# Lumina-Group/libzkp

Hardware: AMD Instinct MI355X
Metric: proofs/sec (whole node) + ms/proof p50, 4096-proof mixed batch (range / equality / membership / improvement) per MI355X (higher is better)
Workload: dtype u32/u64 integer limbs (10x25.5-bit GF(2^255-19), BN254 Fq on 9x29-bit limbs in the MSM loops and 10x26-bit elsewhere, 8x32-bit Fr and scalars mod l, 2x64-bit f128)

## Files before the change

libzkp_amd/csrc/edg.h:

```cpp
#pragma once
#include "bp_steps.h"

namespace zkp {

constexpr uint32_t EDG_WBITS = 16, EDG_NWIN = 16, EDG_NENT = 1u << 15, EDG_DIGW = 8, EDG_NWIN_U64 = 5;
constexpr uint32_t EDG_SLOT_W = 32, EDG_ENTRY_W = 24;
constexpr uint32_t EDG_SEG = 64, EDG_NSEG = EDG_NENT / EDG_SEG, EDG_INV = 8;

struct EdgGeom { uint32_t wbits, nwin, nwin_u64, nent, nseg; };
constexpr uint32_t EDG_WBITS_MIN = 10, EDG_WBITS_MAX = 16;
ZKP_HD constexpr EdgGeom edg_geom(uint32_t wbits) {
    return EdgGeom{wbits, sc_signed_ndigits(wbits, 254), sc_signed_ndigits(wbits, 65), 1u << (wbits - 1), (1u << (wbits - 1)) / EDG_SEG};
}
static_assert(edg_geom(EDG_WBITS).nwin == EDG_NWIN && edg_geom(EDG_WBITS).nwin_u64 == EDG_NWIN_U64 && edg_geom(EDG_WBITS).nent == EDG_NENT &&
              edg_geom(EDG_WBITS).nseg == EDG_NSEG, "the EDG_* constants are the radix-2^16 geometry");
static_assert(edg_geom(EDG_WBITS_MIN).nwin <= 2 * DIGW, "digit rows hold 2 * DIGW digits");
ZKP_HD constexpr size_t edg_table_words(const EdgGeom& g) { return (size_t)NBASE * g.nwin * g.nent * EDG_SLOT_W; }
ZKP_HD constexpr size_t edg_slot(const EdgGeom& g, uint32_t b, uint32_t w, uint32_t e) { return (((size_t)b * g.nwin + w) * g.nent + e) * EDG_SLOT_W; }
ZKP_HD constexpr size_t edg_table_words() { return edg_table_words(edg_geom(EDG_WBITS)); }
ZKP_HD constexpr size_t edg_slot(uint32_t b, uint32_t w, uint32_t e) { return edg_slot(edg_geom(EDG_WBITS), b, w, e); }

ZKP_HD inline ge_niels edg_unpack(const uint32_t e[EDG_ENTRY_W]) {
    ge_niels n; n.ypx = fe_fromwords(e); n.ymx = fe_fromwords(e + 8); n.xy2d = fe_fromwords(e + 16);
    return n;
// ... 36 lines not shown
ZKP_HD inline void edg_step_bases(const uint32_t* gens, uint32_t* bases, uint32_t b) { edg_step_bases(edg_geom(EDG_WBITS), gens, bases, b); }
ZKP_HD inline void edg_step_starts(const uint32_t* bases, uint32_t* starts, uint32_t bw) { edg_step_starts(edg_geom(EDG_WBITS), bases, starts, bw); }
ZKP_HD inline void edg_step_fill(const uint32_t* bases, const uint32_t* starts, uint32_t* table, uint32_t bw, uint32_t s) { edg_step_fill(edg_geom(EDG_WBITS), bases, starts, table, bw, s); }
ZKP_HD inline fe edg_fe_invert(const fe& z) {
    fe t = fe_pow22523(z);
    t = fe_sq(fe_sq(fe_sq(t)));
    return fe_mul(t, fe_mul(fe_sq(z), z));
}
ZKP_HD inline void edg_step_affine(uint32_t* table, size_t group) {
    uint32_t* q0 = table + group * EDG_INV * EDG_SLOT_W;
    fe pre[EDG_INV];
    fe run = fe_one();
    for (uint32_t i = 0; i < EDG_INV; i++) {
        fe z; ZKP_UNROLL for (int k = 0; k < 10; k++) z.v[k] = q0[(size_t)i * EDG_SLOT_W + 20 + k];
        pre[i] = run; run = fe_mul(run, z);
    }
    fe inv = edg_fe_invert(run);
    const fe d2 = fe_const_d2();
    for (uint32_t i = EDG_INV; i-- > 0;) {
        uint32_t* q = q0 + (size_t)i * EDG_SLOT_W;
        fe X, Y, Z; ZKP_UNROLL for (int k = 0; k < 10; k++) { X.v[k] = q[k]; Y.v[k] = q[10 + k]; Z.v[k] = q[20 + k]; }
        const fe zi = fe_mul(inv, pre[i]);
        inv = fe_mul(inv, Z);
        const fe x = fe_mul(X, zi), y = fe_mul(Y, zi);
        fe_towords(q, fe_add(y, x));
        fe_towords(q + 8, fe_sub(y, x));
        fe_towords(q + 16, fe_mul(fe_mul(x, y), d2));
        ZKP_UNROLL for (int k = EDG_ENTRY_W; k < (int)EDG_SLOT_W; k++) q[k] = 0;
    }
}
ZKP_HD inline bool edg_niels_equals(const ge& p, const uint32_t e[EDG_ENTRY_W]) {
    const ge_niels n = edg_unpack(e);
    return fe_eq(fe_add(p.Y, p.X), fe_mul(n.ypx, p.Z)) && fe_eq(fe_sub(p.Y, p.X), fe_mul(n.ymx, p.Z));
}
ZKP_HD inline ge edg_point_of(const uint32_t e[EDG_ENTRY_W]) {
    const ge_niels n = edg_unpack(e);
    ge p; p.X = fe_carry(fe_sub(n.ypx, n.ymx)); p.Y = fe_carry(fe_add(n.ypx, n.ymx)); p.Z = fe_zero(); p.Z.v[0] = 2;
    p.T = fe_mul(p.X, p.Y); p.X = fe_carry(fe_add(p.X, p.X)); p.Y = fe_carry(fe_add(p.Y, p.Y)); p.Z.v[0] = 4;
    return p;
}
ZKP_HD inline bool edg_step_check(const EdgGeom& g, const uint32_t* table, const uint32_t* gens, uint32_t b, uint32_t w, uint32_t e) {
    const uint32_t* cur = table + edg_slot(g, b, w, e);
    if (e + 1 < g.nent) {
        const ge sum = ge_madd(edg_point_of(cur), edg_unpack(table + edg_slot(g, b, w, 0)));
        if (!edg_niels_equals(sum, cur + EDG_SLOT_W)) return false;
    } else if (w + 1 < g.nwin) {
        if (!edg_niels_equals(ge_dbl(edg_point_of(cur)), table + edg_slot(g, b, w + 1, 0))) return false;
    }
    if (w == 0 && e == 0 && !edg_niels_equals(ld_ge(gens, b, 0, 1), cur)) return false;
    return true;
}
ZKP_HD inline bool edg_step_check(const uint32_t* table, const uint32_t* gens, uint32_t b, uint32_t w, uint32_t e) { return edg_step_check(edg_geom(EDG_WBITS), table, gens, b, w, e); }

}
```

libzkp_amd/csrc/edg_kernels.hip:

```cpp
#include "edg_launch.h"
#include "msm_kernel.h"

struct EdGather {
    static constexpr uint32_t ACC_W = GE_W, DIG_PER_WORD = 2;
    static __device__ __forceinline__ int32_t digit(uint32_t word, uint32_t w) { return (int32_t)(int16_t)(word >> (16 * (w & 1u))); }
    using Acc = ge;
    static __device__ __forceinline__ Acc identity() { return ge_identity(); }
    static constexpr uint32_t GATHER_WAVES = 3; static constexpr int GATHER_PREFETCH = 2;
    static constexpr uint32_t GATHER_W = EDG_ENTRY_W, GATHER_STRIDE = EDG_SLOT_W, GATHER_PRIO = 0;
    using GAcc = ge;
    static __device__ __forceinline__ GAcc to_gather(const ge& a) { return a; }
    static __device__ __forceinline__ ge from_gather(const GAcc& a) { return a; }
    static __device__ __forceinline__ GAcc accumulate_entry(const GAcc& acc, int32_t d, const uint32_t* e) { return edg_accumulate(acc, d, e); }
    static __device__ __forceinline__ void store(uint32_t* p, uint32_t idx, uint32_t row, uint32_t rows, const Acc& a) { st_ge(p, idx, row, rows, a); }
    static __device__ __forceinline__ Acc load(const uint32_t* p, uint32_t idx, uint32_t row, uint32_t rows) { return ld_ge(p, idx, row, rows); }
    static __device__ __forceinline__ Acc add(const Acc& a, const Acc& b) { return ge_add(a, b); }
};
template __global__ void k_msm_gather<EdGather>(MsmView, uint32_t, uint32_t);
struct EdGatherPrio : EdGather { static constexpr uint32_t GATHER_PRIO = 1; };
template __global__ void k_msm_gather<EdGatherPrio>(MsmView, uint32_t, uint32_t);

uint32_t edg_msm_rows_per_block() { return 256; }
uint32_t edg_msm_blocks_per_cu() {
    int occ = 0;
    if (hipOccupancyMaxActiveBlocksPerMultiprocessor(&occ, k_msm_gather<EdGather>, 256, gather_lds_bytes<EdGather>()) != hipSuccess) { (void)hipGetLastError(); return 0; }
    return occ > 0 ? (uint32_t)occ : 0;
}
void edg_launch_msm(const MsmView& m, uint32_t ngroups, uint32_t nblocks, hipStream_t st, bool raised) {
    const uint32_t grid = ((nblocks + 7) / 8) * 8;
    if (raised) k_msm_gather<EdGatherPrio><<<grid, 256, gather_lds_bytes<EdGather>(), st>>>(m, ngroups, nblocks);
    else k_msm_gather<EdGather><<<grid, 256, gather_lds_bytes<EdGather>(), st>>>(m, ngroups, nblocks);
}

template <uint32_t WB> __global__ void __launch_bounds__(64) k_edg_bases(const uint32_t* gens, uint32_t* bases) {
    const uint32_t b = blockIdx.x * 64 + threadIdx.x;
    if (b < NBASE) edg_step_bases(edg_geom(WB), gens, bases, b);
}
template <uint32_t WB> __global__ void __launch_bounds__(64) k_edg_starts(const uint32_t* bases, uint32_t* starts) {
    constexpr EdgGeom g = edg_geom(WB);
    const uint32_t bw = blockIdx.x * 64 + threadIdx.x;
    if (bw < NBASE * g.nwin) edg_step_starts(g, bases, starts, bw);
}
template <uint32_t WB> __global__ void __launch_bounds__(256) k_edg_fill(const uint32_t* bases, const uint32_t* starts, uint32_t* table) {
    constexpr EdgGeom g = edg_geom(WB);
    const uint32_t t = blockIdx.x * 256 + threadIdx.x;
    if (t < NBASE * g.nwin * g.nseg) edg_step_fill(g, bases, starts, table, t / g.nseg, t % g.nseg);
}
template <uint32_t WB> __global__ void __launch_bounds__(256) k_edg_affine(uint32_t* table) {
    constexpr EdgGeom g = edg_geom(WB);
    const size_t grp = (size_t)blockIdx.x * 256 + threadIdx.x;
    if (grp < (size_t)NBASE * g.nwin * g.nent / EDG_INV) edg_step_affine(table, grp);
}
template <uint32_t WB> __global__ void __launch_bounds__(256) k_edg_check(const uint32_t* table, const uint32_t* gens, int* bad) {
    constexpr EdgGeom g = edg_geom(WB);
    const size_t t = (size_t)blockIdx.x * 256 + threadIdx.x;
    if (t >= (size_t)NBASE * g.nwin * g.nent) return;
    const uint32_t e = (uint32_t)(t % g.nent), bw = (uint32_t)(t / g.nent);
    if (!edg_step_check(g, table, gens, bw / g.nwin, bw % g.nwin, e)) atomicAdd(bad, 1);
}
template <uint32_t WB> void edg_launch_build_at(const uint32_t* d_gens, uint32_t* d_table, uint32_t* d_scratch, int* d_bad, hipStream_t st) {
    constexpr EdgGeom g = edg_geom(WB);
    uint32_t* bases = d_scratch;
    uint32_t* starts = d_scratch + (size_t)NBASE * g.nwin * GE_W;
    k_edg_bases<WB><<<(NBASE + 63) / 64, 64, 0, st>>>(d_gens, bases);
    k_edg_starts<WB><<<(NBASE * g.nwin + 63) / 64, 64, 0, st>>>(bases, starts);
    k_edg_fill<WB><<<(NBASE * g.nwin * g.nseg + 255) / 256, 256, 0, st>>>(bases, starts, d_table);
    const size_t groups = (size_t)NBASE * g.nwin * g.nent / EDG_INV, slots = (size_t)NBASE * g.nwin * g.nent;
    k_edg_affine<WB><<<(uint32_t)((groups + 255) / 256), 256, 0, st>>>(d_table);
    k_edg_check<WB><<<(uint32_t)((slots + 255) / 256), 256, 0, st>>>(d_table, d_gens, d_bad);
}
size_t edg_build_scratch_words(const EdgGeom& g) { return (size_t)NBASE * g.nwin * (g.nseg + 1) * GE_W; }
void edg_launch_build(const EdgGeom& g, const uint32_t* d_gens, uint32_t* d_table, uint32_t* d_scratch, int* d_bad, hipStream_t st) {
    switch (g.wbits) {
        case 10: edg_launch_build_at<10>(d_gens, d_table, d_scratch, d_bad, st); break;
        case 11: edg_launch_build_at<11>(d_gens, d_table, d_scratch, d_bad, st); break;
        case 12: edg_launch_build_at<12>(d_gens, d_table, d_scratch, d_bad, st); break;
        case 13: edg_launch_build_at<13>(d_gens, d_table, d_scratch, d_bad, st); break;
        case 14: edg_launch_build_at<14>(d_gens, d_table, d_scratch, d_bad, st); break;
        case 15: edg_launch_build_at<15>(d_gens, d_table, d_scratch, d_bad, st); break;
        default: edg_launch_build_at<16>(d_gens, d_table, d_scratch, d_bad, st); break;
    }
}
```

libzkp_amd/csrc/edg_launch.h:

```cpp
#pragma once
#include <hip/hip_runtime.h>
#include "edg.h"

uint32_t edg_msm_rows_per_block();
uint32_t edg_msm_blocks_per_cu();
void edg_launch_msm(const zkp::MsmView& m, uint32_t ngroups, uint32_t nblocks, hipStream_t st, bool raised = false);
void edg_launch_build(const zkp::EdgGeom& g, const uint32_t* d_gens, uint32_t* d_table, uint32_t* d_scratch, int* d_bad, hipStream_t st);
size_t edg_build_scratch_words(const zkp::EdgGeom& g);
void edg_launch_sum(const zkp::ReduceView& R, uint32_t* sums, hipStream_t st);
```

libzkp_amd/csrc/zkp_hip.hip:

```cpp
#include <hip/hip_runtime.h>
#include <mutex>
#include <memory>
#include <algorithm>
#include <map>
#include <array>
#include <type_traits>
#include <atomic>
#include <thread>
#include <condition_variable>
#include <functional>
#include <deque>
#include <new>
#include <exception>
#include <cstring>
#include <string>
#include <vector>
#include <cstdio>
#include <cstdlib>
#include <cmath>
#include <chrono>
#include <sys/random.h>
#include "bp_layout.h"
#include "g16_steps.h"
#include "sha256_host.h"
// ... 201 lines not shown
    std::vector<void*> owned;
    DevScope() = default;
    DevScope(const DevScope&) = delete;
    DevScope& operator=(const DevScope&) = delete;
    ~DevScope() { release(); }
    void release() { if (!owned.empty()) dev_scope_quiesce(); for (void* q : owned) dev_pool().give(q); owned.clear(); }
    template <class T> hipError_t alloc(T** out, size_t bytes) {
        void* q = nullptr;
        const hipError_t e = dev_pool().take(&q, bytes ? bytes : 1);
        if (e == hipSuccess) owned.push_back(q);
        *out = static_cast<T*>(q);
        return e;
    }
};
struct Quiesce { bool armed = true; ~Quiesce() { if (armed) (void)hipDeviceSynchronize(); } };

struct DevLayout {
    uint16_t *slot_base = nullptr, *chunk_begin = nullptr, *chunk_win0 = nullptr, *chunk_nwin = nullptr, *target_chunk_begin = nullptr;
    uint8_t* slot_nwin = nullptr;
    uint32_t nslots = 0, nchunks = 0, ntargets = 0, max_chunk_windows = 0, max_target_chunks = 0;
    uint64_t adds_per_row = 0;
    uint32_t *steps = nullptr, *chunk_step0 = nullptr;
};
constexpr int MAXT = 8;
struct LayoutSet { std::vector<DevLayout> cand; uint32_t max_chunks = 0; };

struct SubBatch {
    hipStream_t stream = nullptr;
    hipEvent_t start = nullptr, done = nullptr;
    hipStream_t side = nullptr;
    hipEvent_t side_go = nullptr, side_done = nullptr;
    bool used = false;
    bool borrowed = false;
    void* ws = nullptr;
    uint32_t capM = 0, capC = 0, cap_chunks = 0;
};
constexpr uint32_t NSLOTS = 2;

struct G16State; struct StarkState; struct VfyState; struct BatchState;
struct Device {
    int index = 0, hip_dev = 0;
    std::mutex mu;
    bool ready = false;
    uint64_t generation = 0;
    int num_cu = 256;
    int msm_prio_now = 0;
    hipStream_t stream = nullptr;
    uint32_t* d_edg_table = nullptr;
    EdgGeom edg = {0, 0, 0, 0, 0};
    bool bp_ready = false;
    int edg_blocks_per_cu = 3;
    struct Family { LayoutSet p1, rd[6]; bool ready = false; };
    Family fam[4];
    LayoutSet p2, ct;
    uint32_t max_chunks = 0;
    SubBatch sub[NSLOTS];
    uint32_t next_slot = 0;
    DevPool pool;
    G16State* g16 = nullptr; StarkState* stark = nullptr; VfyState* vfy = nullptr; BatchState* batch = nullptr;
    bool profiling = false;
    struct KProf {
        std::vector<std::pair<hipEvent_t, hipEvent_t>> ev_pool; size_t ev_used = 0;
        double ms = 0; uint64_t launches = 0, adds = 0;
    };
    KProf prof[3];
    struct HostCounter { double ms = 0; uint64_t a = 0, b = 0; };
    HostCounter host[ZKP_HIP_COUNTER_VERIFY_MIXED - ZKP_HIP_COUNTER_G16_VERIFY + 1];
    HostCounter& counter(int which) { return host[which - ZKP_HIP_COUNTER_G16_VERIFY]; }
    struct BpLocaliseCounter { double ms = 0; uint64_t failed_checks = 0, segment_checks = 0, jobs_again = 0; } bp_localise;
    struct CompositesCounter { double ms = 0; uint64_t composites = 0, malformed = 0, envelopes = 0; } composites;
    uint64_t stark_verify_resident = 0;
    struct Trace* trace = nullptr;
    struct ShardWorker* worker = nullptr;
};
struct ShardWorker {
    struct Job { std::function<void()> fn; bool done = false; };
    using Ticket = std::shared_ptr<Job>;
    std::mutex mu; std::condition_variable cv;
    std::deque<Ticket> queue;
    std::thread th;
    ShardWorker() : th([this]() { run(); }) { th.detach(); }
    void run() {
        for (;;) {
            Ticket t;
            { std::unique_lock<std::mutex> lk(mu); cv.wait(lk, [this]() { return !queue.empty(); }); t = queue.front(); queue.pop_front(); }
            t->fn();
            { std::lock_guard<std::mutex> lk(mu); t->done = true; }
            cv.notify_all();
        }
    }
    Ticket post(std::function<void()> f) {
        Ticket t = std::make_shared<Job>(); t->fn = std::move(f);
        { std::lock_guard<std::mutex> lk(mu); queue.push_back(t); }
        cv.notify_all();
        return t;
    }
    void wait(const Ticket& t) { std::unique_lock<std::mutex> lk(mu); cv.wait(lk, [&]() { return t->done; }); }
};
std::mutex g_worker_create_mu;
int prof_begin(Device::KProf& K, hipStream_t st, hipEvent_t* e1);
void prof_end(Device::KProf& K, hipStream_t st, hipEvent_t e1, uint64_t adds);
struct Registry {
    std::mutex mu;
    std::vector<Device*> shards;
    bool hooked = false;
};
Registry& registry() { static Registry* r = new Registry(); return *r; }
thread_local Device* t_dev = nullptr;
thread_local int t_sel = 0;
thread_local bool t_sel_chosen = false;
Device& dev() { return *t_dev; }
DevPool& dev_pool() { return dev().pool; }
void dev_scope_quiesce() { if (dev().stream) (void)hipStreamSynchronize(dev().stream); }
uint32_t g_budget_request = 0;
int env_int(const char* name, int dflt) { const char* v = getenv(name); return v && *v ? atoi(v) : dflt; }
int stream_priority(int level) {
    int least = 0, greatest = 0; (void)hipDeviceGetStreamPriorityRange(&least, &greatest);
    return level == 0 ? greatest : level == 2 ? least : (least + greatest) / 2;
}
int bp_priority_level() { static const int v = env_int("ZKP_HIP_BP_PRIORITY", 1); return v; }
int stark_priority_level() { static const int v = env_int("ZKP_HIP_STARK_PRIORITY", 1); return v; }
int g16_priority_level() { static const int v = env_int("ZKP_HIP_G16_PRIORITY", 2); return v; }

int prof_begin(Device::KProf& K, hipStream_t st, hipEvent_t* e1) {
    *e1 = nullptr;
    if (!dev().profiling) return 0;
    if (K.ev_used == K.ev_pool.size()) { hipEvent_t a, b; HIP_TRY(hipEventCreate(&a)); HIP_TRY(hipEventCreate(&b)); K.ev_pool.push_back({a, b}); }
    HIP_TRY(hipEventRecord(K.ev_pool[K.ev_used].first, st));
    *e1 = K.ev_pool[K.ev_used].second; K.ev_used++;
    return 0;
}
void prof_end(Device::KProf& K, hipStream_t st, hipEvent_t e1, uint64_t adds) {
    if (!e1) return;
    (void)hipEventRecord(e1, st); K.launches++; K.adds += adds;
}

struct Trace {
    struct Rec { const char* name; hipStream_t st; hipEvent_t a, b; };
    std::vector<Rec> recs;
    std::vector<hipEvent_t> pool; size_t used = 0;
    hipEvent_t origin = nullptr; bool have_origin = false;
    std::string path;
    hipEvent_t take() { if (used == pool.size()) { hipEvent_t e = nullptr; (void)hipEventCreate(&e); pool.push_back(e); } return pool[used++]; }
};
Trace* trace_state() {
    Device& D = dev();
    if (D.trace) return D.trace->path.empty() ? nullptr : D.trace;
    D.trace = new Trace();
    const char* v = getenv("ZKP_HIP_TRACE");
    if (v && *v) D.trace->path = v;
    return D.trace->path.empty() ? nullptr : D.trace;
}
void trace_origin(hipStream_t st) {
    Trace* T = trace_state(); if (!T) return;
    if (!T->origin) (void)hipEventCreate(&T->origin);
    (void)hipEventRecord(T->origin, st); T->have_origin = true;
}
struct TraceMark {
    Trace* T; Trace::Rec r;
    TraceMark(const char* name, hipStream_t st) : T(trace_state()) { if (T) { r = {name, st, T->take(), T->take()}; (void)hipEventRecord(r.a, st); } }
    ~TraceMark() { if (T) { (void)hipEventRecord(r.b, r.st); T->recs.push_back(r); } }
};
#define ZKP_TRACED(name, st, ...) do { TraceMark tm_(name, st); __VA_ARGS__; } while (0)
void trace_dump() {
    Trace* T = trace_state(); if (!T || T->recs.empty()) return;
    (void)hipDeviceSynchronize();
    FILE* f = fopen(T->path.c_str(), "a");
    if (f) {
        std::map<hipStream_t, int> ids;
        fputs("[", f);
        bool first = true;
        for (auto& r : T->recs) {
            float ta = 0, tb = 0;
            if (!T->have_origin || hipEventElapsedTime(&ta, T->origin, r.a) != hipSuccess || hipEventElapsedTime(&tb, T->origin, r.b) != hipSuccess) continue;
            const int id = ids.emplace(r.st, (int)ids.size()).first->second;
// ... 144 lines not shown
    if (!strcmp(v, "lazy")) { *lazy = true; return 0; }
    return fail(ZKP_HIP_E_ARGUMENT, "ZKP_HIP_ED_TABLES must be eager or lazy");
}
int build_edg_table() {
    Device& D = dev();
    if (D.d_edg_table) return 0;
    EdgTables& R = edg_tables();
    std::lock_guard<std::mutex> registry_lock(R.mu);
    {
        const uint32_t occ = edg_msm_blocks_per_cu();
        D.edg_blocks_per_cu = occ ? (int)occ : 3;
    }
    for (auto& e : R.v) if (e.hip_dev == D.hip_dev && e.refs > 0) { e.refs++; D.d_edg_table = e.table; D.edg = e.geom; return 0; }
    uint32_t wbits = 0;
    int rc = choose_ed_radix(&wbits);
    if (rc) return rc;
    const EdgGeom g = edg_geom(wbits);
    ge gens[NBASE]; host_generators(gens);
    std::vector<uint32_t> gw((size_t)NBASE * GE_W);
    for (uint32_t b = 0; b < NBASE; b++) st_ge(gw.data(), b, 0, 1, gens[b]);
    uint32_t *d_gens = nullptr, *d_scratch = nullptr; int* d_bad = nullptr;
    const size_t table_bytes = edg_table_words(g) * 4, scratch_bytes = edg_build_scratch_words(g) * 4;
    if (hipMalloc(&D.d_edg_table, table_bytes) != hipSuccess) {
        (void)hipGetLastError(); D.d_edg_table = nullptr;
        char msg[200]; snprintf(msg, sizeof msg, "out of device memory allocating the %llu MB of generator window tables (radix 2^%u)", (unsigned long long)(table_bytes >> 20), wbits);
        return fail(ZKP_HIP_E_RUNTIME, msg);
    }
    auto drop = [&]() { (void)hipFree(d_gens); (void)hipFree(d_scratch); (void)hipFree(d_bad); };
    auto give_up = [&](int code, const std::string& m) { drop(); (void)hipFree(D.d_edg_table); D.d_edg_table = nullptr; return fail(code, m); };
    hipError_t e = hipMalloc(&d_gens, gw.size() * 4);
    if (e == hipSuccess) e = hipMalloc(&d_scratch, scratch_bytes);
    if (e == hipSuccess) e = hipMalloc(&d_bad, sizeof(int));
    if (e == hipSuccess) e = hipMemcpyAsync(d_gens, gw.data(), gw.size() * 4, hipMemcpyHostToDevice, D.stream);
    if (e == hipSuccess) e = hipMemsetAsync(d_bad, 0, sizeof(int), D.stream);
    if (e != hipSuccess) return give_up(ZKP_HIP_E_RUNTIME, std::string("generator tables: ") + hipGetErrorString(e));
    edg_launch_build(g, d_gens, D.d_edg_table, d_scratch, d_bad, D.stream);
    int bad = -1;
    e = hipGetLastError();
    if (e == hipSuccess) e = hipMemcpyAsync(&bad, d_bad, sizeof(int), hipMemcpyDeviceToHost, D.stream);
    if (e == hipSuccess) e = hipStreamSynchronize(D.stream);
    if (e != hipSuccess) return give_up(ZKP_HIP_E_RUNTIME, std::string("generator tables: ") + hipGetErrorString(e));
    if (bad != 0) { char msg[160]; snprintf(msg, sizeof msg, "generator window tables failed their self-check (%d inconsistent slots)", bad); return give_up(ZKP_HIP_E_RUNTIME, msg); }
    drop();
    D.edg = g;
    R.v.push_back({D.hip_dev, D.d_edg_table, 1, g});
    return 0;
}
int ensure_bp() {
    Device& D = dev();
    if (D.bp_ready) return 0;
    int rc;
    if ((rc = build_edg_table())) return rc;
    D.max_chunks = 0;
    if ((rc = upload_set(D.p2, targets_phase2((uint8_t)D.edg.nwin)))) return rc;
    if ((rc = upload_set(D.ct, targets_ctask((uint8_t)D.edg.nwin, (uint8_t)D.edg.nwin_u64)))) return rc;
    D.max_chunks = D.p2.max_chunks;
    if ((rc = ensure_family(6))) return rc;
    D.bp_ready = true;
    return 0;
}

int init_device() {
    Device& D = dev();
    if (D.ready) return 0;
    bool lazy = false;
    int rc = ed_tables_lazy(&lazy);
    if (rc) return rc;
    hipDeviceProp_t prop; HIP_TRY(hipGetDeviceProperties(&prop, D.hip_dev));
    D.num_cu = prop.multiProcessorCount > 0 ? prop.multiProcessorCount : 256;
    if (!D.stream) HIP_TRY(hipStreamCreateWithFlags(&D.stream, hipStreamNonBlocking));
    if (!lazy && (rc = ensure_bp())) return rc;
    D.ready = true;
    return 0;
}
void release_sub(SubBatch& sb) {
    if (sb.ws) (void)hipFree(sb.ws);
    for (hipEvent_t e : {sb.start, sb.done, sb.side_go, sb.side_done}) if (e) (void)hipEventDestroy(e);
    if (!sb.borrowed) { if (sb.stream) (void)hipStreamDestroy(sb.stream); if (sb.side) (void)hipStreamDestroy(sb.side); }
    sb = SubBatch();
}
int ensure_sub(SubBatch& sb, SubBatch* share = nullptr) {
    if (sb.stream) return 0;
    SubBatch t;
    int rc = 0;
    if (share && share != &sb) {
        if ((rc = ensure_sub(*share))) return rc;
        t.stream = share->stream; t.side = share->side; t.borrowed = true;
    } else {
        hipError_t e = hipStreamCreateWithPriority(&t.stream, hipStreamNonBlocking, stream_priority(bp_priority_level()));
        if (e == hipSuccess) e = hipStreamCreateWithPriority(&t.side, hipStreamNonBlocking, stream_priority(bp_priority_level()));
        if (e != hipSuccess) { release_sub(t); return fail(ZKP_HIP_E_RUNTIME, std::string("hipStreamCreateWithPriority: ") + hipGetErrorString(e)); }
    }
    for (hipEvent_t* e : {&t.start, &t.done, &t.side_go, &t.side_done}) {
        const hipError_t err = hipEventCreateWithFlags(e, hipEventDisableTiming);
        if (err != hipSuccess) { *e = nullptr; release_sub(t); return fail(ZKP_HIP_E_RUNTIME, std::string("hipEventCreateWithFlags: ") + hipGetErrorString(err)); }
    }
    sb.start = t.start; sb.done = t.done; sb.side_go = t.side_go; sb.side_done = t.side_done;
    sb.side = t.side; sb.borrowed = t.borrowed; sb.stream = t.stream;
    return 0;
}

extern "C" void zkp_hip_shutdown(void);
void batch_release_all();
void stark_release_all();
int register_shards_locked(Registry& R, const int* devices, uint32_t count, bool add, const char* bad_index) {
    int ndev = 0;
    if (hipGetDeviceCount(&ndev) != hipSuccess || ndev == 0)
        return fail(ZKP_HIP_E_RUNTIME, "zkp_hip_init: no HIP device available (this library has no CPU fallback)");
    for (uint32_t k = 0; k < count; k++) if (devices[k] < 0 || devices[k] >= ndev) return fail(ZKP_HIP_E_ARGUMENT, bad_index);
// ... 100 lines not shown
        rc = verify_fan_out(shards, F.holds.empty() ? nullptr : F.holds.data(), n, F.prefix.empty() ? nullptr : F.prefix.data(), F.unit, F.min_jobs, slice, &fanned);
        if (rc || fanned) return rc;
    }
    Bind bind;
    if ((rc = bind.open())) return rc;
    return slice(0, n);
}
struct EnvelopeUpload {
    DevScope mem;
    uint8_t *d_in = nullptr, *d_ok = nullptr; uint32_t* d_len = nullptr; uint64_t *d_p0 = nullptr, *d_p1 = nullptr;
    int open(uint64_t n, const uint8_t* proofs, uint64_t stride, const uint32_t* lens, const uint64_t* p0 = nullptr, const uint64_t* p1 = nullptr) {
        hipStream_t st = dev().stream;
        HIP_TRY(mem.alloc(&d_in, stride * n)); HIP_TRY(mem.alloc(&d_len, 4 * n)); HIP_TRY(mem.alloc(&d_ok, n));
        if (p0) HIP_TRY(mem.alloc(&d_p0, 8 * n));
        if (p1) HIP_TRY(mem.alloc(&d_p1, 8 * n));
        HIP_TRY(hipMemcpyAsync(d_in, proofs, stride * n, hipMemcpyHostToDevice, st));
        HIP_TRY(hipMemcpyAsync(d_len, lens, 4 * n, hipMemcpyHostToDevice, st));
        if (p0) HIP_TRY(hipMemcpyAsync(d_p0, p0, 8 * n, hipMemcpyHostToDevice, st));
        if (p1) HIP_TRY(hipMemcpyAsync(d_p1, p1, 8 * n, hipMemcpyHostToDevice, st));
        return 0;
    }
};

struct Ws {
    JobBuf J; BpView V; CtView T;
    uint32_t *partial, *ct_partial, *ct_enc, *sums, *ct_sums;
    uint64_t* ct_off;
    int* flag;
};
size_t align_up(size_t x) { return (x + 255) & ~(size_t)255; }

size_t carve(uint8_t* base, uint32_t M, uint32_t C, uint32_t max_chunks, Ws* w) {
    size_t off = 0;
    auto take = [&](size_t bytes) { uint8_t* p = base ? base + off : nullptr; off += align_up(bytes); return p; };
    const size_t W = (size_t)8 * 4 * M;
    const size_t WD = (size_t)DIGW * 4 * M;
    Ws t{};
    t.J.v = (uint64_t*)take(8ull * M); t.J.seed_ix = (uint32_t*)take(4ull * M); t.J.proof_ix = (uint32_t*)take(4ull * M);
    t.J.bl_plus = (int32_t*)take(4ull * M); t.J.bl_minus = (int32_t*)take(4ull * M); t.J.kind = (uint8_t*)take(M);
    t.J.proof_off = (uint64_t*)take(8ull * M); t.J.commit_off = (uint64_t*)take(8ull * M);
    t.J.ct_v = (uint64_t*)take(8ull * C); t.J.ct_seed_ix = (uint32_t*)take(4ull * C); t.J.ct_bl_ix = (uint32_t*)take(4ull * C); t.J.ct_off = (uint64_t*)take(8ull * C);
    t.V.wbits = dev().edg.wbits; t.T.wbits = dev().edg.wbits;
    t.V.M = M; t.V.v = t.J.v; t.V.seed_ix = t.J.seed_ix; t.V.proof_ix = t.J.proof_ix; t.V.bl_plus = t.J.bl_plus; t.V.bl_minus = t.J.bl_minus;
    t.V.kind = t.J.kind; t.V.proof_off = t.J.proof_off; t.V.commit_off = t.J.commit_off;
    t.V.tape = (uint32_t*)take(W * TAPE_SLOTS); t.V.gamma = (uint32_t*)take(W);
    t.V.d1 = (uint32_t*)take(WD * P1_NSLOTS); t.V.d2 = (uint32_t*)take(WD * P2_NSLOTS); t.V.dr = (uint32_t*)take(WD * PR_NSLOTS);
    t.V.yinvpow = (uint32_t*)take(W * 64); t.V.ypq = (uint32_t*)take(W * 32); t.V.r0 = (uint32_t*)take(W * 64); t.V.r1 = (uint32_t*)take(W * 64);
    t.V.pp = (uint32_t*)take(W * 192); t.V.ab = (uint32_t*)take(W * 256); t.V.gh = (uint32_t*)take(W * 128);
    t.V.scal = (uint32_t*)take(W * SC_NUM); t.V.tstate = (uint32_t*)take(4ull * 52 * M); t.V.enc = (uint32_t*)take(W * 3);
    t.partial = (uint32_t*)take((size_t)max_chunks * GE_W * 4 * M);
    t.sums = (uint32_t*)take((size_t)3 * GE_W * 4 * M);
    t.T.C = C; t.T.v = t.J.ct_v; t.T.seed_ix = t.J.ct_seed_ix; t.T.bl_ix = t.J.ct_bl_ix;
    t.T.digits = (uint32_t*)take((size_t)2 * DIGW * 4 * C);
    t.ct_partial = (uint32_t*)take((size_t)(dev().ct.max_chunks ? dev().ct.max_chunks : 2) * GE_W * 4 * C);
    t.ct_enc = (uint32_t*)take((size_t)8 * 4 * C);
    t.ct_sums = (uint32_t*)take((size_t)GE_W * 4 * C);
    t.ct_off = t.J.ct_off;
    t.flag = (int*)take(256);
    if (w) *w = t;
    return off;
}

int ensure_workspace(SubBatch& sb, uint32_t M, uint32_t C) {
    if (M <= sb.capM && C <= sb.capC && dev().max_chunks <= sb.cap_chunks && sb.ws) return 0;
    if (sb.ws) { HIP_TRY(hipDeviceSynchronize()); HIP_TRY(hipFree(sb.ws)); sb.ws = nullptr; }
    const uint32_t nm = M > sb.capM ? M : sb.capM, nc = C > sb.capC ? C : sb.capC;
    const size_t bytes = carve(nullptr, nm, nc, dev().max_chunks, nullptr);
    HIP_TRY(hipMalloc(&sb.ws, bytes));
    sb.capM = nm; sb.capC = nc; sb.cap_chunks = dev().max_chunks;
    return 0;
}

int launch_msm(const DevLayout& D, uint32_t rows, const uint32_t* digits, uint32_t* partial, hipStream_t st) {
    MsmView m; m.rows = rows; m.nslots = D.nslots; m.nchunks = D.nchunks; m.table = dev().d_edg_table; m.digits = digits;
    m.slot_base = D.slot_base; m.slot_scalar = nullptr; m.slot_nwin = D.slot_nwin; m.chunk_begin = D.chunk_begin; m.chunk_win0 = D.chunk_win0; m.chunk_nwin = D.chunk_nwin; m.partial = partial; m.acc_init = nullptr;
    hipEvent_t e1 = nullptr;
    int rc = prof_begin(dev().prof[0], st, &e1);
    if (rc) return rc;
    {
        const EdgGeom& g = dev().edg;
        m.nwin = g.nwin; m.nent = g.nent; m.digw = DIGW; m.slot_ent = g.nwin * g.nent; m.uneven = 0;
        m.steps = D.steps; m.chunk_step0 = D.chunk_step0;
        const uint32_t tb = edg_msm_rows_per_block(), ngroups = (rows + tb - 1) / tb, nblocks = D.nchunks * ngroups;
        ZKP_TRACED("k_msm_gather<EdGather>", st, edg_launch_msm(m, ngroups, nblocks, st, dev().msm_prio_now != 0));
    }
    prof_end(dev().prof[0], st, e1, D.adds_per_row * rows);
    return 0;
}
void launch_sum_ed(const ReduceView& R, uint32_t* sums, hipStream_t st) {
    k_sum_t<EdMsm, ED_SUM_ROWS, ED_SUM_TB><<<dim3((R.rows + ED_SUM_ROWS - 1) / ED_SUM_ROWS, R.ntargets), ED_SUM_TB, 0, st>>>(R, sums);
}
int launch_reduce(const DevLayout& D, uint32_t rows, const uint32_t* partial, uint32_t* sums, uint32_t* enc, const uint64_t* out_off, uint8_t* out, hipStream_t st) {
    ReduceView R; R.rows = rows; R.ntargets = D.ntargets; R.partial = partial; R.target_chunk_begin = D.target_chunk_begin;
    R.enc = enc; R.out_off = out_off; R.out = out; R.corr = nullptr;
    ZKP_TRACED("k_sum_t<EdMsm>", st, launch_sum_ed(R, sums, st));
    ZKP_TRACED("k_encode", st, k_encode<<<dim3((rows + TW - 1) / TW, D.ntargets), TW, 0, st>>>(R, sums));
    return 0;
}
int msm_and_encode(const LayoutSet& S, uint32_t rows, const uint32_t* digits, uint32_t* partial, uint32_t* sums, uint32_t* enc, const uint64_t* out_off, uint8_t* out, hipStream_t st) {
    const DevLayout& D = pick_layout(S, rows);
    int rc = launch_msm(D, rows, digits, partial, st);
    if (rc) return rc;
    return launch_reduce(D, rows, partial, sums, enc, out_off, out, st);
}

int run_pipeline(const Ws& w, uint32_t M, uint32_t C, hipStream_t st, SubBatch& lane) {
    int rc;
    const dim3 gj((M + TB - 1) / TB), gw((M + TW - 1) / TW);
    const uint32_t n = w.V.n, lg = w.V.lg;
    const Device::Family& F = dev().fam[lg - 3];
    const bool forked = C != 0 && M != 0;
    if (C) {
        hipStream_t cs = forked ? lane.side : st;
        if (forked) { HIP_TRY(hipEventRecord(lane.side_go, st)); HIP_TRY(hipStreamWaitEvent(cs, lane.side_go, 0)); }
        ZKP_TRACED("k_ctask", cs, k_ctask<<<(C + TB - 1) / TB, TB, 0, cs>>>(w.T));
        if ((rc = msm_and_encode(dev().ct, C, w.T.digits, w.ct_partial, w.ct_sums, w.ct_enc, w.ct_off, w.V.out, cs))) return rc;
        if (forked) HIP_TRY(hipEventRecord(lane.side_done, cs));
    }
    if (M == 0) { HIP_TRY(hipGetLastError()); return 0; }
    ZKP_TRACED("k_tape", st, k_tape<<<dim3(gj.x, tape_slots(n) + 1), TB, 0, st>>>(w.V));
    if ((rc = msm_and_encode(F.p1, M, w.V.d1, w.partial, w.sums, w.V.enc, nullptr, nullptr, st))) return rc;
    ZKP_TRACED("k_transcript1", st, k_transcript1<<<gw, TW, 0, st>>>(w.V));
    ZKP_TRACED("k_poly", st, k_poly<<<dim3(gj.x, n), TB, 0, st>>>(w.V));
    ZKP_TRACED("k_poly_sum", st, k_poly_sum<<<(M + 7) / 8, TW, 0, st>>>(w.V));
    if ((rc = msm_and_encode(dev().p2, M, w.V.d2, w.partial, w.sums, w.V.enc, nullptr, nullptr, st))) return rc;
    ZKP_TRACED("k_transcript2", st, k_transcript2<<<gw, TW, 0, st>>>(w.V));
    ZKP_TRACED("k_lr_init", st, k_lr_init<<<dim3(gj.x, n), TB, 0, st>>>(w.V));
    for (uint32_t r = 0; r < lg; r++) {
        ZKP_TRACED("k_round_prep", st, k_round_prep<<<dim3(gj.x, n), TB, 0, st>>>(w.V, r));
        ZKP_TRACED("k_round_sum", st, k_round_sum<<<gw, TW, 0, st>>>(w.V, r));
        if ((rc = msm_and_encode(F.rd[r], M, w.V.dr, w.partial, w.sums, w.V.enc, nullptr, nullptr, st))) return rc;
        ZKP_TRACED("k_transcript_round", st, k_transcript_round<<<gw, TW, 0, st>>>(w.V, r));
    }
    if (forked) HIP_TRY(hipStreamWaitEvent(st, lane.side_done, 0));
    HIP_TRY(hipGetLastError());
    return 0;
}

__global__ void k_any_failed(const int32_t* status, uint32_t n, int* flag) {
    const uint32_t i = blockIdx.x * blockDim.x + threadIdx.x;
    if (i < n && status[i] != 0) atomicOr(flag, 1);
}

int prove_range_device_locked(uint64_t n, const uint64_t* d_value, const uint64_t* d_min, const uint64_t* d_max, uint32_t lg,
                              const uint8_t* d_seeds, uint8_t* d_out, uint64_t stride, uint32_t* d_out_len, int32_t* d_status,
                              hipStream_t st, int* any_failed, int slot_hint = -1) {
    if (n == 0) { if (any_failed) *any_failed = 0; return 0; }
    { int rcn = check_batch_size(n); if (rcn) return rcn; }
    if (stride < range_envelope_bytes(lg)) return fail(ZKP_HIP_E_ARGUMENT, "stride is smaller than the proof (1478 bytes for n_bits = 64)");
    int rc;
    if ((rc = ensure_family(lg))) return rc;
    uint32_t slot = 0;
    if (slot_hint >= 0) slot = (uint32_t)slot_hint % NSLOTS;
    else {
        SubBatch& s0 = dev().sub[0];
        if (s0.used && hipEventQuery(s0.done) == hipErrorNotReady) { slot = 1 + dev().next_slot % (NSLOTS - 1); dev().next_slot++; }
        (void)hipGetLastError();
    }
    SubBatch& sb = dev().sub[slot];
    if ((rc = ensure_sub(sb, &dev().sub[0]))) return rc;
    HIP_TRY(hipEventRecord(sb.start, st));
    const uint32_t C = (uint32_t)n, M = 2 * C;
    if ((rc = ensure_workspace(sb, M, C))) return rc;
    Ws w; carve((uint8_t*)sb.ws, M, C, dev().max_chunks, &w);
    w.V.n = 1u << lg; w.V.lg = lg;
    w.V.seeds = reinterpret_cast<const uint32_t*>(d_seeds); w.T.seeds = w.V.seeds;
    w.V.out = d_out;
    HIP_TRY(hipStreamWaitEvent(sb.stream, sb.start, 0));
    if (sb.used) HIP_TRY(hipStreamWaitEvent(sb.stream, sb.done, 0));
    ZKP_TRACED("k_build_range", sb.stream, k_build_range<<<(C + TB - 1) / TB, TB, 0, sb.stream>>>(w.J, C, d_value, d_min, d_max, lg, w.V.out, stride, d_out_len, d_status));
    if ((rc = run_pipeline(w, M, C, sb.stream, sb))) return rc;
    HIP_TRY(hipEventRecord(sb.done, sb.stream)); sb.used = true;
    HIP_TRY(hipStreamWaitEvent(st, sb.done, 0));
    if (any_failed) {
        Ws wf; carve((uint8_t*)sb.ws, sb.capM, sb.capC, dev().max_chunks, &wf);
        HIP_TRY(hipMemsetAsync(wf.flag, 0, sizeof(int), st));
        k_any_failed<<<(uint32_t)((n + TB - 1) / TB), TB, 0, st>>>(d_status, (uint32_t)n, wf.flag);
        HIP_TRY(hipMemcpyAsync(any_failed, wf.flag, sizeof(int), hipMemcpyDeviceToHost, st));
// ... 292 lines not shown
```

Before: 347,400.

## Compute small two-base products with a dedicated fused gather-accumulate-encode kernel

Replaces the generic chunked MSM plus reduce plus encode path for the phase-2 commitments and the ctask commitments, which each touch only two fixed bases, with one kernel. In it, 4 lanes per row each walk a strided subset of windows, prefetch table entries two steps ahead, combine partial sums through wave shuffles, and Ristretto-encode directly. This removes the partial-sum buffers, the separate sum and encode launches, and the per-target layout uploads. In exchange it uses fewer threads per product and relies on per-lane prefetch rather than the cooperative LDS gather. It can be turned off with an environment variable.

```diff
diff --git a/libzkp_amd/csrc/edg.h b/libzkp_amd/csrc/edg.h
--- a/libzkp_amd/csrc/edg.h
+++ b/libzkp_amd/csrc/edg.h
@@ -112,4 +112,54 @@
 }
 ZKP_HD inline bool edg_step_check(const uint32_t* table, const uint32_t* gens, uint32_t b, uint32_t w, uint32_t e) { return edg_step_check(edg_geom(EDG_WBITS), table, gens, b, w, e); }
 
+struct EdgSmallTarget { uint32_t base0, nwin0, drow0, base1, nwin1, drow1; };
+constexpr uint32_t EDG_SMALL_LANES = 4;
+constexpr int EDG_SMALL_LEAD = 2;
+struct alignas(16) EdgQuad { uint32_t w[4]; };
+static_assert(EDG_ENTRY_W % 4 == 0 && EDG_SLOT_W % 4 == 0, "entries are whole 16-byte pieces");
+ZKP_HD inline ge edg_small_part(const EdgGeom& g, const uint32_t* table, const uint32_t* digits, uint32_t rows, uint32_t row,
+                                const EdgSmallTarget& t, uint32_t part, uint32_t nparts) {
+    constexpr int LEAD = EDG_SMALL_LEAD; constexpr uint32_t V4 = EDG_ENTRY_W / 4;
+    const uint32_t total = t.nwin0 + t.nwin1;
+    const uint32_t nsteps = row < rows && part < total ? (total - part + nparts - 1) / nparts : 0;
+    auto digit_of = [&](uint32_t i) -> int32_t {
+        const uint32_t k = part + i * nparts; const bool second = k >= t.nwin0;
+        return i < nsteps ? ld_digit(digits, second ? t.drow1 : t.drow0, second ? k - t.nwin0 : k, row, rows) : 0;
+    };
+    auto fetch = [&](EdgQuad* dst, uint32_t i, int32_t d) {
+        if (d == 0) return;
+        const uint32_t k = part + i * nparts; const bool second = k >= t.nwin0;
+        const EdgQuad* src = reinterpret_cast<const EdgQuad*>(table + edg_slot(g, second ? t.base1 : t.base0, second ? k - t.nwin0 : k, (uint32_t)(d < 0 ? -d : d) - 1));
+        ZKP_UNROLL for (uint32_t v = 0; v < V4; v++) dst[v] = src[v];
+    };
+    EdgQuad e[LEAD + 1][V4]; int32_t dd[LEAD + 1];
+    ZKP_UNROLL for (int j = 0; j < LEAD; j++) { dd[j] = digit_of((uint32_t)j); fetch(e[j], (uint32_t)j, dd[j]); }
+    int32_t q0 = digit_of(LEAD), q1 = digit_of(LEAD + 1);
+    ge acc = ge_identity();
+    for (uint32_t i = 0; i < nsteps; i++) {
+        dd[LEAD] = q0; fetch(e[LEAD], i + LEAD, q0);
+        q0 = q1; q1 = digit_of(i + LEAD + 2);
+        if (dd[0] != 0) acc = edg_accumulate(acc, dd[0], reinterpret_cast<const uint32_t*>(e[0]));
+        ZKP_UNROLL for (int j = 0; j < LEAD; j++) { ZKP_UNROLL for (uint32_t v = 0; v < V4; v++) e[j][v] = e[j + 1][v]; dd[j] = dd[j + 1]; }
+    }
+    return acc;
 }
+ZKP_HD inline ge edg_small_join(const ge* parts, uint32_t nparts) {
+    ge s[EDG_SMALL_LANES];
+    for (uint32_t p = 0; p < nparts; p++) s[p] = parts[p];
+    for (uint32_t stride = 1; stride < nparts; stride <<= 1) {
+        ge n[EDG_SMALL_LANES];
+        for (uint32_t p = 0; p < nparts; p++) n[p] = ge_add(s[p], s[p ^ stride]);
+        for (uint32_t p = 0; p < nparts; p++) s[p] = n[p];
+    }
+    return s[0];
+}
+ZKP_HD inline void edg_small_store(const ge& sum, uint32_t* enc, uint32_t target, uint32_t row, uint32_t rows, const uint64_t* out_off, uint8_t* out) {
+    sc e; ge_ristretto_encode(e.v, sum);
+    st_sc(enc, target, row, rows, e);
+    if (out_off != nullptr && target == 0) put_bytes(out + out_off[row], e.v, 8);
+}
+ZKP_HD inline EdgSmallTarget edg_small_phase2(const EdgGeom& g, uint32_t target) { return EdgSmallTarget{BASE_B, g.nwin, 2 * target, BASE_BB, g.nwin, 2 * target + 1}; }
+ZKP_HD inline EdgSmallTarget edg_small_ctask(const EdgGeom& g) { return EdgSmallTarget{BASE_B, g.nwin_u64, 0, BASE_BB, g.nwin, 1}; }
+
+}
diff --git a/libzkp_amd/csrc/edg_kernels.hip b/libzkp_amd/csrc/edg_kernels.hip
--- a/libzkp_amd/csrc/edg_kernels.hip
+++ b/libzkp_amd/csrc/edg_kernels.hip
@@ -30,6 +30,38 @@
     const uint32_t grid = ((nblocks + 7) / 8) * 8;
     if (raised) k_msm_gather<EdGatherPrio><<<grid, 256, gather_lds_bytes<EdGather>(), st>>>(m, ngroups, nblocks);
     else k_msm_gather<EdGather><<<grid, 256, gather_lds_bytes<EdGather>(), st>>>(m, ngroups, nblocks);
+}
+
+struct EdgSmallView {
+    EdgGeom g; const uint32_t* table; const uint32_t* digits; uint32_t rows, ntargets;
+    EdgSmallTarget t0, t1;
+    uint32_t* enc; const uint64_t* out_off; uint8_t* out;
+};
+__device__ __forceinline__ ge small_exchange(const ge& a, int stride) {
+    ge o;
+    ZKP_UNROLL for (int k = 0; k < 10; k++) {
+        o.X.v[k] = (uint32_t)__shfl_xor((int)a.X.v[k], stride, 64); o.Y.v[k] = (uint32_t)__shfl_xor((int)a.Y.v[k], stride, 64);
+        o.Z.v[k] = (uint32_t)__shfl_xor((int)a.Z.v[k], stride, 64); o.T.v[k] = (uint32_t)__shfl_xor((int)a.T.v[k], stride, 64);
+    }
+    return o;
+}
+__global__ void __launch_bounds__(64) k_small_products(EdgSmallView v) {
+    ZKP_RAISE_PRIO();
+    constexpr uint32_t PER_WAVE = 64 / EDG_SMALL_LANES;
+    const uint32_t part = threadIdx.x % EDG_SMALL_LANES, p = blockIdx.x * PER_WAVE + threadIdx.x / EDG_SMALL_LANES;
+    const bool active = p < v.rows * v.ntargets;
+    const uint32_t target = active ? p / v.rows : 0, row = active ? p % v.rows : v.rows;
+    const EdgSmallTarget t = target == 0 ? v.t0 : v.t1;
+    ge acc = edg_small_part(v.g, v.table, v.digits, v.rows, row, t, part, EDG_SMALL_LANES);
+    ZKP_UNROLL for (int stride = 1; stride < (int)EDG_SMALL_LANES; stride <<= 1) acc = ge_add(acc, small_exchange(acc, stride));
+    if (active && part == 0) edg_small_store(acc, v.enc, target, row, v.rows, v.out_off, v.out);
+}
+void edg_launch_small_products(const EdgGeom& g, const uint32_t* table, const uint32_t* digits, uint32_t rows, uint32_t ntargets, const EdgSmallTarget* targets,
+                               uint32_t* enc, const uint64_t* out_off, uint8_t* out, hipStream_t st) {
+    if (rows == 0 || ntargets == 0) return;
+    EdgSmallView v{g, table, digits, rows, ntargets, targets[0], targets[ntargets > 1 ? 1 : 0], enc, out_off, out};
+    constexpr uint32_t PER_WAVE = 64 / EDG_SMALL_LANES;
+    k_small_products<<<(uint32_t)(((uint64_t)rows * ntargets + PER_WAVE - 1) / PER_WAVE), 64, 0, st>>>(v);
 }
 
 template <uint32_t WB> __global__ void __launch_bounds__(64) k_edg_bases(const uint32_t* gens, uint32_t* bases) {
diff --git a/libzkp_amd/csrc/edg_launch.h b/libzkp_amd/csrc/edg_launch.h
--- a/libzkp_amd/csrc/edg_launch.h
+++ b/libzkp_amd/csrc/edg_launch.h
@@ -5,6 +5,8 @@
 uint32_t edg_msm_rows_per_block();
 uint32_t edg_msm_blocks_per_cu();
 void edg_launch_msm(const zkp::MsmView& m, uint32_t ngroups, uint32_t nblocks, hipStream_t st, bool raised = false);
+void edg_launch_small_products(const zkp::EdgGeom& g, const uint32_t* table, const uint32_t* digits, uint32_t rows, uint32_t ntargets, const zkp::EdgSmallTarget* targets,
+                               uint32_t* enc, const uint64_t* out_off, uint8_t* out, hipStream_t st);
 void edg_launch_build(const zkp::EdgGeom& g, const uint32_t* d_gens, uint32_t* d_table, uint32_t* d_scratch, int* d_bad, hipStream_t st);
 size_t edg_build_scratch_words(const zkp::EdgGeom& g);
 void edg_launch_sum(const zkp::ReduceView& R, uint32_t* sums, hipStream_t st);
diff --git a/libzkp_amd/csrc/zkp_hip.hip b/libzkp_amd/csrc/zkp_hip.hip
--- a/libzkp_amd/csrc/zkp_hip.hip
+++ b/libzkp_amd/csrc/zkp_hip.hip
@@ -277,6 +277,7 @@
     int edg_blocks_per_cu = 3;
     struct Family { LayoutSet p1, rd[6]; bool ready = false; };
     Family fam[4];
+    bool small_products = true;
     LayoutSet p2, ct;
     uint32_t max_chunks = 0;
     SubBatch sub[NSLOTS];
@@ -346,6 +347,7 @@
 int bp_priority_level() { static const int v = env_int("ZKP_HIP_BP_PRIORITY", 1); return v; }
 int stark_priority_level() { static const int v = env_int("ZKP_HIP_STARK_PRIORITY", 1); return v; }
 int g16_priority_level() { static const int v = env_int("ZKP_HIP_G16_PRIORITY", 2); return v; }
+bool bp_small_products() { return dev().small_products; }
 
 int prof_begin(Device::KProf& K, hipStream_t st, hipEvent_t* e1) {
     *e1 = nullptr;
@@ -596,9 +598,12 @@
     int rc;
     if ((rc = build_edg_table())) return rc;
     D.max_chunks = 0;
-    if ((rc = upload_set(D.p2, targets_phase2((uint8_t)D.edg.nwin)))) return rc;
-    if ((rc = upload_set(D.ct, targets_ctask((uint8_t)D.edg.nwin, (uint8_t)D.edg.nwin_u64)))) return rc;
-    D.max_chunks = D.p2.max_chunks;
+    D.small_products = env_int("ZKP_HIP_BP_SMALL_PRODUCTS", 1) != 0;
+    if (!D.small_products) {
+        if ((rc = upload_set(D.p2, targets_phase2((uint8_t)D.edg.nwin)))) return rc;
+        if ((rc = upload_set(D.ct, targets_ctask((uint8_t)D.edg.nwin, (uint8_t)D.edg.nwin_u64)))) return rc;
+        D.max_chunks = D.p2.max_chunks;
+    }
     if ((rc = ensure_family(6))) return rc;
     D.bp_ready = true;
     return 0;
@@ -805,9 +810,11 @@
     t.sums = (uint32_t*)take((size_t)3 * GE_W * 4 * M);
     t.T.C = C; t.T.v = t.J.ct_v; t.T.seed_ix = t.J.ct_seed_ix; t.T.bl_ix = t.J.ct_bl_ix;
     t.T.digits = (uint32_t*)take((size_t)2 * DIGW * 4 * C);
-    t.ct_partial = (uint32_t*)take((size_t)(dev().ct.max_chunks ? dev().ct.max_chunks : 2) * GE_W * 4 * C);
     t.ct_enc = (uint32_t*)take((size_t)8 * 4 * C);
-    t.ct_sums = (uint32_t*)take((size_t)GE_W * 4 * C);
+    if (!bp_small_products()) {
+        t.ct_partial = (uint32_t*)take((size_t)(dev().ct.max_chunks ? dev().ct.max_chunks : 2) * GE_W * 4 * C);
+        t.ct_sums = (uint32_t*)take((size_t)GE_W * 4 * C);
+    }
     t.ct_off = t.J.ct_off;
     t.flag = (int*)take(256);
     if (w) *w = t;
@@ -856,6 +863,9 @@
     if (rc) return rc;
     return launch_reduce(D, rows, partial, sums, enc, out_off, out, st);
 }
+void small_products(uint32_t rows, uint32_t ntargets, const EdgSmallTarget* targets, const uint32_t* digits, uint32_t* enc, const uint64_t* out_off, uint8_t* out, hipStream_t st) {
+    ZKP_TRACED("k_small_products", st, edg_launch_small_products(dev().edg, dev().d_edg_table, digits, rows, ntargets, targets, enc, out_off, out, st));
+}
 
 int run_pipeline(const Ws& w, uint32_t M, uint32_t C, hipStream_t st, SubBatch& lane) {
     int rc;
@@ -867,7 +877,8 @@
         hipStream_t cs = forked ? lane.side : st;
         if (forked) { HIP_TRY(hipEventRecord(lane.side_go, st)); HIP_TRY(hipStreamWaitEvent(cs, lane.side_go, 0)); }
         ZKP_TRACED("k_ctask", cs, k_ctask<<<(C + TB - 1) / TB, TB, 0, cs>>>(w.T));
-        if ((rc = msm_and_encode(dev().ct, C, w.T.digits, w.ct_partial, w.ct_sums, w.ct_enc, w.ct_off, w.V.out, cs))) return rc;
+        if (bp_small_products()) { const EdgSmallTarget t = edg_small_ctask(dev().edg); small_products(C, 1, &t, w.T.digits, w.ct_enc, w.ct_off, w.V.out, cs); }
+        else if ((rc = msm_and_encode(dev().ct, C, w.T.digits, w.ct_partial, w.ct_sums, w.ct_enc, w.ct_off, w.V.out, cs))) return rc;
         if (forked) HIP_TRY(hipEventRecord(lane.side_done, cs));
     }
     if (M == 0) { HIP_TRY(hipGetLastError()); return 0; }
@@ -876,7 +887,8 @@
     ZKP_TRACED("k_transcript1", st, k_transcript1<<<gw, TW, 0, st>>>(w.V));
     ZKP_TRACED("k_poly", st, k_poly<<<dim3(gj.x, n), TB, 0, st>>>(w.V));
     ZKP_TRACED("k_poly_sum", st, k_poly_sum<<<(M + 7) / 8, TW, 0, st>>>(w.V));
-    if ((rc = msm_and_encode(dev().p2, M, w.V.d2, w.partial, w.sums, w.V.enc, nullptr, nullptr, st))) return rc;
+    if (bp_small_products()) { const EdgSmallTarget t[2] = {edg_small_phase2(dev().edg, 0), edg_small_phase2(dev().edg, 1)}; small_products(M, 2, t, w.V.d2, w.V.enc, nullptr, nullptr, st); }
+    else if ((rc = msm_and_encode(dev().p2, M, w.V.d2, w.partial, w.sums, w.V.enc, nullptr, nullptr, st))) return rc;
     ZKP_TRACED("k_transcript2", st, k_transcript2<<<gw, TW, 0, st>>>(w.V));
     ZKP_TRACED("k_lr_init", st, k_lr_init<<<dim3(gj.x, n), TB, 0, st>>>(w.V));
     for (uint32_t r = 0; r < lg; r++) {
```

After: 350,200, median of 3. About the same (+0.8%).
